# GinZhu/RDST

Hardware: AMD Instinct MI355X
Metric: SR patches/sec fwd+bwd, RDST-E1 x4 64->256 (higher is better)
Workload: dtype bf16; 1 GPU; RDST-E1 x4 (RDST_E1_OASIS_example_SRx4.ini), 1x64x64 LR patches -> 256x256, step = fwd + L1 + bwd + flat-bucket grad all-reduce + Adam; global_batch=32, per_gpu_batch=32, parallelism=dp1, hip_graph=True, grad_bucket_bytes=17859844

## Files before the change

rdst_amd/csrc/lin3_mfma.hip:

```cpp
#include "linear.h"
#include "lds_dma.h"
#include "mfma.h"
#include "pack.h"

namespace {

constexpr int L3_TT = 128;

__global__ void __launch_bounds__(256) lin3_pack_kernel(const float* __restrict__ W, const float* __restrict__ gamma,
                                                        const float* __restrict__ beta, const float* __restrict__ bias,
                                                        bf16* __restrict__ wp, float* __restrict__ sb, int N, int K, int ksteps,
                                                        int ntiles, float s) {
  lin3_pack_block((int)blockIdx.x, W, gamma, beta, bias, wp, sb, N, K, ksteps, ntiles, s);
}

struct L3Args {
  const bf16* X; int64_t ldx; int x_bytes;
  const bf16* Wp; const float* sb;
  const bf16* R; int64_t ldr; int r_bytes;
  bf16* Y; int64_t ldy;
  float* stats;
  int M, N, ntiles;
};

constexpr int l3_nw(int NT) { return (NT >= 4 && NT <= 12) ? NT : 8; }

template <int K, int NT, bool LN, bool RES>
struct L3Cfg {
  static constexpr int KSTEPS = (K + 15) / 16;
  static constexpr int XS = lds_kstep_stride(K), XSLOTS = XS / 16, XD = (2 * K + 15) / 16;
  static constexpr int TP = (L3_TT * XSLOTS + 63) / 64, TILEB = TP * 1024;
  static constexpr int RS = RES ? NT * 64 + 16 : 0, RSLOTS = RS / 16, RP = RES ? (L3_TT * RSLOTS + 63) / 64 : 0, RTILEB = RP * 1024;
  static constexpr int WGCU = l3_nw(NT) > 8 ? 1 : 2;
  static constexpr int NBUF = RES ? 1 : (WGCU == 1 ? 4 : 2);
  static constexpr int NW = l3_nw(NT);
  static constexpr int NTHR = 64 * NW;
  static constexpr int ITEMS = NT * 4, NJ = (ITEMS + NW - 1) / NW;
  static constexpr int PERIOD = NT / ce_gcd(NW, NT), ND = NJ < PERIOD ? NJ : PERIOD;
  static constexpr int CNT = (TP + NW - 1) / NW + (RES ? (RP + NW - 1) / NW : 0);
  static constexpr int R_OFF = NBUF * TILEB;
  static constexpr int STAT_OFF = R_OFF + NBUF * RTILEB;
  static constexpr int SB_OFF = STAT_OFF + NBUF * L3_TT * 2 * 4;
  static constexpr int SMEM = SB_OFF + (2 * NT * 32 * 4 + 1023) / 1024 * 1024;
  static_assert(SMEM <= 160 * 1024, "LDS");
  static_assert(CNT * (NBUF - 1) < 64, "vmcnt is a 6-bit counter");
  static_assert(TP >= NW && (!RES || RP >= NW), "every wave owns at least one piece of a tile");
};

template <int K, int NT, bool LN, bool RES>
__global__ void __launch_bounds__(64 * l3_nw(NT), l3_nw(NT) > 8 ? 1 : (2 * l3_nw(NT) + 3) / 4) lin3_kernel(const L3Args p) {
  using CF = L3Cfg<K, NT, LN, RES>;
  constexpr int KSTEPS = CF::KSTEPS, XS = CF::XS, NBUF = CF::NBUF, ND = CF::ND, NJ = CF::NJ, NW = CF::NW, NTHR = CF::NTHR;
  extern __shared__ __attribute__((aligned(16))) char smem[];
  const int tid = threadIdx.x, lane = tid & 63, r = lane & 31, h = lane >> 5;
  const int wave = __builtin_amdgcn_readfirstlane(tid >> 6);
  float* statL = reinterpret_cast<float*>(smem + CF::STAT_OFF);
  const float* sbL = reinterpret_cast<const float*>(smem + CF::SB_OFF);

  const u32x4s_t rsx = dma_rsrc(p.X, (uint32_t)p.x_bytes), rsr = dma_rsrc(RES ? (const void*)p.R : (const void*)p.X, (uint32_t)p.r_bytes),
                 rsb = dma_rsrc(p.sb, 2 * NT * 32 * 4);
  const uint32_t lds0 = lds_base(smem);
  const int grid = gridDim.x;
  u32x4v_t wfr[ND][KSTEPS];
#pragma unroll
  for (int jd = 0; jd < ND; ++jd) {
    const int nt = (wave + NW * jd) % NT;
#pragma unroll
    for (int ks = 0; ks < KSTEPS; ++ks) {
      const char* src = reinterpret_cast<const char*>(p.Wp) + (((int64_t)nt * KSTEPS + ks) * 64 + lane) * 16;
      frag_load(wfr[jd][ks], src);
    }
  }
  {
    constexpr int NSBP = (2 * NT * 32 * 4 + 1023) / 1024;
    const int pc = wave % NSBP;
    lds_dma16(rsb, __builtin_amdgcn_readfirstlane(lds0 + (uint32_t)(CF::SB_OFF + pc * 1024)), pc * 1024 + lane * 16);
  }
  constexpr int CNT = CF::CNT;
  auto issue_round = [&](int tile0) {
#pragma unroll
    for (int b = 0; b < NBUF; ++b) {
      const int tile = tile0 + b * grid;
#pragma unroll
      for (int i = 0; i < (CF::TP + NW - 1) / NW; ++i) {
        int q = wave + NW * i;
        q = q < CF::TP ? q : q - NW;
        const int sidx = q * 64 + lane;
        const int tok = sidx / CF::XSLOTS, sl = sidx - tok * CF::XSLOTS;
        const int grow = tile * L3_TT + tok;
        const bool ok = tile < p.ntiles && tok < L3_TT && sl < CF::XD && grow < p.M;
        lds_dma16(rsx, __builtin_amdgcn_readfirstlane(lds0 + (uint32_t)(b * CF::TILEB + q * 1024)),
            ok ? grow * ((int)p.ldx * 2) + sl * 16 : p.x_bytes);
      }
      if constexpr (RES) {
#pragma unroll
        for (int i = 0; i < (CF::RP + NW - 1) / NW; ++i) {
          int q = wave + NW * i;
          q = q < CF::RP ? q : q - NW;
          const int sidx = q * 64 + lane;
          const int tok = sidx / CF::RSLOTS, sl = sidx - tok * CF::RSLOTS;
          const int grow = tile * L3_TT + tok;
          const bool ok = tile < p.ntiles && tok < L3_TT && sl * 8 < p.N && grow < p.M;
          lds_dma16(rsr, __builtin_amdgcn_readfirstlane(lds0 + (uint32_t)(CF::R_OFF + b * CF::RTILEB + q * 1024)),
              ok ? grow * ((int)p.ldr * 2) + sl * 16 : p.r_bytes);
        }
      }
    }
  };

  for (int tile0 = blockIdx.x; tile0 < p.ntiles; tile0 += grid * NBUF) {
    issue_round(tile0);
#pragma unroll 1
    for (int b = 0; b < NBUF; ++b) {
      const int tile = tile0 + b * grid;
      if (tile >= p.ntiles) break;
      switch (NBUF - 1 - b) {
        case 3: wait_vmcnt<CNT * 3>(); break;
        case 2: wait_vmcnt<CNT * 2>(); break;
        case 1: wait_vmcnt<CNT * 1>(); break;
        default: wait_vmcnt<0>(); break;
      }
#pragma unroll
      for (int jd = 0; jd < ND; ++jd)
#pragma unroll
        for (int ks = 0; ks < KSTEPS; ++ks) frag_pin(wfr[jd][ks]);
      __syncthreads();
      const char* tb = smem + b * CF::TILEB;
      const char* rb = smem + CF::R_OFF + b * CF::RTILEB;
      float* st = statL + b * L3_TT * 2;
      if constexpr (LN) {
        for (int tok = tid >> 2; tok < L3_TT; tok += NTHR / 4) {
          const int part = tid & 3;
          constexpr int NSL = (CF::XD + 3) / 4;
          float xv[NSL][8];
          float sum = 0.f;
#pragma unroll
          for (int i = 0; i < NSL; ++i) {
            const int sl = part + 4 * i;
            const Pack16 q = *reinterpret_cast<const Pack16*>(tb + tok * XS + (sl < CF::XD ? sl : 0) * 16);
            Mma<bf16>::unpack(q, xv[i]);
#pragma unroll
            for (int e = 0; e < 8; ++e) {
              const bool valid = sl < CF::XD && sl * 8 + e < K;
              xv[i][e] = valid ? xv[i][e] : 0.f;
              sum += xv[i][e];
            }
          }
          sum += __shfl_xor(sum, 1, 64);
          sum += __shfl_xor(sum, 2, 64);
          const float mean = sum * (1.0f / K);
          float sq = 0.f;
#pragma unroll
          for (int i = 0; i < NSL; ++i) {
            const int sl = part + 4 * i;
#pragma unroll
            for (int e = 0; e < 8; ++e) {
              const bool valid = sl < CF::XD && sl * 8 + e < K;
              const float d = xv[i][e] - mean;
              sq = valid ? fmaf(d, d, sq) : sq;
            }
          }
          sq += __shfl_xor(sq, 1, 64);
          sq += __shfl_xor(sq, 2, 64);
          const float rstd = rsqrtf(sq * (1.0f / K) + 1e-5f);
          if (part == 0) {
            st[tok * 2] = mean;
            st[tok * 2 + 1] = rstd;
            const int grow = tile * L3_TT + tok;
            if (grow < p.M) *reinterpret_cast<float2*>(p.stats + (int64_t)grow * 2) = make_float2(mean, rstd);
          }
        }
        __syncthreads();
      }
#pragma unroll
      for (int jd = 0; jd < ND; ++jd)
#pragma unroll 1
      for (int j = jd; j < NJ; j += ND) {
        const int item = wave + NW * j;
        if (item >= CF::ITEMS) break;
        const int nt = item % NT, tt = item / NT;
        const int tok = tt * 32 + r;
        const int grow = tile * L3_TT + tok;
        f32x16 acc;
#pragma unroll
        for (int v = 0; v < 16; ++v) acc[v] = 0.f;
        const char* brow = tb + tok * XS + h * 16;
#pragma unroll
        for (int ks = 0; ks < KSTEPS; ++ks) {
          Pack16 bq = *reinterpret_cast<const Pack16*>(brow + ks * 32);
          if (K % 16 != 0 && ks == KSTEPS - 1) {
            constexpr int c0 = K % 16 < 8 ? K % 16 : 8, c1 = K % 16 > 8 ? K % 16 - 8 : 0;
#pragma unroll
            for (int d = 0; d < 4; ++d) bq.w[d] = (2 * d < (h ? c1 : c0)) ? bq.w[d] : 0u;
          }
          acc = __builtin_amdgcn_mfma_f32_32x32x16_bf16(__builtin_bit_cast(bf16x8_t, wfr[jd][ks]), __builtin_bit_cast(bf16x8_t, bq), acc, 0, 0, 0);
        }
        float mean = 0.f, rstd = 1.f;
        if constexpr (LN) {
          const float2 mr = *reinterpret_cast<const float2*>(st + tok * 2);
          mean = mr.x; rstd = mr.y;
        }
        const float nrm = -rstd * mean;
#pragma unroll
        for (int g4 = 0; g4 < 4; ++g4) {
          const int n0 = nt * 32 + 8 * g4 + 4 * h;
          const float4 S4 = *reinterpret_cast<const float4*>(sbL + n0);
          const float4 B4 = *reinterpret_cast<const float4*>(sbL + NT * 32 + n0);
          if constexpr (LN) {
            acc[4 * g4] = fmaf(rstd, acc[4 * g4], fmaf(nrm, S4.x, B4.x));
            acc[4 * g4 + 1] = fmaf(rstd, acc[4 * g4 + 1], fmaf(nrm, S4.y, B4.y));
            acc[4 * g4 + 2] = fmaf(rstd, acc[4 * g4 + 2], fmaf(nrm, S4.z, B4.z));
            acc[4 * g4 + 3] = fmaf(rstd, acc[4 * g4 + 3], fmaf(nrm, S4.w, B4.w));
          } else {
            acc[4 * g4] += B4.x; acc[4 * g4 + 1] += B4.y; acc[4 * g4 + 2] += B4.z; acc[4 * g4 + 3] += B4.w;
          }
          if constexpr (RES) {
            const u32x2_a4 rr = *reinterpret_cast<const u32x2_a4*>(rb + tok * CF::RS + n0 * 2);
            acc[4 * g4] += bf16lo(rr.x); acc[4 * g4 + 1] += bf16hi(rr.x);
            acc[4 * g4 + 2] += bf16lo(rr.y); acc[4 * g4 + 3] += bf16hi(rr.y);
          }
        }
        if (grow < p.M) {
#pragma unroll
          for (int gp = 0; gp < 2; ++gp) {
            float c8[8];
#pragma unroll
            for (int e = 0; e < 4; ++e) {
              const auto sw = __builtin_amdgcn_permlane32_swap(__float_as_uint(acc[8 * gp + e]), __float_as_uint(acc[8 * gp + 4 + e]),
                                                               false, false);
              c8[e] = __uint_as_float(sw[0]);
              c8[4 + e] = __uint_as_float(sw[1]);
            }
            const int cb = nt * 32 + 8 * (2 * gp + h);
            const int nv = p.N - cb;
            if (nv <= 0) continue;
            bf16* yp = p.Y + (grow * (int)p.ldy + cb);
            if (nv >= 8) {
              u32x4_a4 u;
              u.x = pack_bf16x2(c8[0], c8[1]); u.y = pack_bf16x2(c8[2], c8[3]);
              u.z = pack_bf16x2(c8[4], c8[5]); u.w = pack_bf16x2(c8[6], c8[7]);
              *reinterpret_cast<u32x4_a4*>(yp) = u;
            } else {
#pragma unroll
              for (int d = 0; d < 3; ++d)
                if (2 * d + 2 <= nv) *reinterpret_cast<uint32_t*>(yp + 2 * d) = pack_bf16x2(c8[2 * d], c8[2 * d + 1]);
            }
          }
        }
      }
    }
    __syncthreads();
  }
}

template <int K, int NT, bool LN, bool RES>
int launch_l3(L3Args& p, hipStream_t st, const char* what) {
  using CF = L3Cfg<K, NT, LN, RES>;
  p.ntiles = (p.M + L3_TT - 1) / L3_TT;
  int grid = (p.ntiles + CF::NBUF - 1) / CF::NBUF;
  if (grid > 256 * CF::WGCU) grid = 256 * CF::WGCU;
  auto kern = lin3_kernel<K, NT, LN, RES>;
  return rdst_launch(kern, dim3((unsigned)grid), dim3(CF::NTHR), CF::SMEM, st, what, p);
}

}

int lin3_pack_launch(const float* W, const float* gamma, const float* beta, const float* bias, void* out, int N, int K, float s,
                     hipStream_t st) {
  const int nt = (N + 31) / 32, ks = (K + 15) / 16;
  bf16* wp = reinterpret_cast<bf16*>(out);
  float* sb = reinterpret_cast<float*>(reinterpret_cast<char*>(out) + (size_t)nt * ks * 1024);
  const int nfr = nt * ks * 64, nb1 = (nfr + 255) / 256, nb2 = (nt * 32 + 3) / 4;
  hipLaunchKernelGGL(lin3_pack_kernel, dim3((unsigned)(nb1 + nb2)), dim3(256), 0, st, W, gamma, beta, bias, wp, sb, N, K, ks, nt, s);
  return rdst_launch_status("lin3_pack");
}

size_t lin3_pack_bytes(int K, int N) {
  const int nt = (N + 31) / 32, ks = (K + 15) / 16;
  return (size_t)nt * ks * 1024 + (size_t)2 * nt * 32 * 4 + 256;
}

int lin3_kind(int K, int N, bool ln, bool res, int in_act) {
  if (in_act || !(K == 60 || K == 90 || K == 120)) return 0;
  if (ln && !res && N == 3 * K) return 1;
  if (!ln && res && N == K) return 2;
  if (ln && !res && N == 30) return 3;
  return 0;
}

int lin3_fwd_bf16(const bf16* X, int64_t ldx, const float* ln_w, const float* ln_b, int in_act, const float* Wt, const float* bias,
                  const bf16* R, int64_t ldr, bf16* Y, int64_t ldy, float* stats, int64_t M, int K, int N, float s, void* wpack,
                  bool prepacked, hipStream_t st) {
  if (!wpack || ((uintptr_t)wpack & 15) || !Wt || M <= 0) return RDST_ENOTSUP;
  const int kind = lin3_kind(K, N, ln_w != nullptr, R != nullptr, in_act);
  if (!kind) return RDST_ENOTSUP;
  if (((uintptr_t)X & 3) || (ldx & 1) || ((uintptr_t)Y & 3) || (ldy & 1) || (R && (((uintptr_t)R & 3) || (ldr & 1)))) return RDST_ENOTSUP;
  const int64_t xb = ((M - 1) * ldx + K) * 2;
  if (xb >= (1ll << 31) || M * ldy * 2 >= (1ll << 31) || (R && M * ldr * 2 >= (1ll << 31))) return RDST_ENOTSUP;
  const int nt = (N + 31) / 32, ks = (K + 15) / 16;
  bf16* wp = reinterpret_cast<bf16*>(wpack);
  float* sb = reinterpret_cast<float*>(reinterpret_cast<char*>(wpack) + (size_t)nt * ks * 1024);
  if (!prepacked)
    if (int rc = lin3_pack_launch(Wt, ln_w, ln_b, bias, wpack, N, K, s, st)) return rc;
  L3Args p{};
  p.X = X; p.ldx = ldx; p.x_bytes = (int)xb; p.Wp = wp; p.sb = sb; p.R = R; p.ldr = ldr;
  p.r_bytes = R ? (int)(((M - 1) * ldr + N) * 2) : 0; p.Y = Y; p.ldy = ldy; p.stats = stats;
  p.M = (int)M; p.N = N;
#define L3_CASE(KK)                                                                                   \
  if (K == KK) {                                                                                      \
    if (kind == 1) return launch_l3<KK, (3 * KK + 31) / 32, true, false>(p, st, "lin3_qkv");           \
    if (kind == 2) return launch_l3<KK, (KK + 31) / 32, false, true>(p, st, "lin3_proj");              \
    return launch_l3<KK, 1, true, false>(p, st, "lin3_tail");                                          \
  }
  L3_CASE(60) L3_CASE(90) L3_CASE(120)
#undef L3_CASE
  return RDST_ENOTSUP;
}
```

rdst_amd/csrc/linear.h:

```cpp
#pragma once
#include "common.h"

template <typename T>
int linear_fwd_mfma(const T* X, int64_t ldx, const float* ln_w, const float* ln_b, int in_act, const float* Wt,
                    const float* bias, const T* R, int64_t ldr, T* Y, int64_t ldy, float* stats, int64_t M, int K,
                    int N, float s, bool split, hipStream_t st);
template <typename T>
int linear_dgrad_mfma(const T* X, int64_t ldx, bool has_ln, int in_act, const float* Wt, const T* dY, int64_t lddy,
                      T* dX, int64_t lddx, const T* acc, int64_t ldacc, float* dA, int64_t M, int K, int N, float s,
                      bool split, hipStream_t st);
template <typename T>
int linear_wgrad_mfma(const T* X, int64_t ldx, const float* ln_w, const float* ln_b, const float* stats, int in_act,
                      const T* dY, int64_t lddy, float* dW, float* dbias, const WsSlab& slab, int64_t M, int K, int N, float s,
                      bool split, hipStream_t st);

constexpr int kLinWgradSplits = 96;
inline int linear_wgrad_max_wgs(int N) { return N <= 128 ? 4 * kCUs : N <= 192 ? 2 * kCUs : kCUs; }
struct LinBwdWs {
  float* dA;
  float* G;
  WsSlab slabW;
  WsSlab small;
  size_t bytes;
};
inline LinBwdWs lin_bwd_layout(void* base, int64_t M, int K, int N, bool ln, bool linear) {
  WsCarver c(base);
  LinBwdWs w{};
  const size_t g = (size_t)N * (K + 1), da = ln ? (size_t)M * K : 0;
  w.dA = c.take<float>(da);
  w.G = ln && linear && g <= da ? w.dA : nullptr;
  const int64_t rows = linear ? linear_wgrad_max_wgs(N) : 0;
  const size_t gen = linear ? (size_t)kLinWgradSplits * N * K : 0, per_wg = (size_t)rows * g;
  w.slabW = WsSlab{c.take<float>(gen > per_wg ? gen : per_wg), rows, (int64_t)g};
  w.small = ws_take_slab(c, kSmallBlocks, N > 2 * K ? N : 2 * K);
  c.take<float>(2 * (size_t)K + kWsSlackFloats);
  w.bytes = c.bytes();
  return w;
}

template <typename T>
int linear_dgrad_ln_mfma(const T* X, int64_t ldx, const float* stats, const float* gamma, const float* Wt, const T* dY,
                         int64_t lddy, T* dX, int64_t lddx, const T* acc, int64_t ldacc, const WsSlab& slab, int* nslab,
                         int64_t M, int K, int N, float s, hipStream_t st);
template <typename T>
int linear_wgrad_ln_mfma(const T* X, int64_t ldx, const float* ln_w, const float* ln_b, const float* stats, const float* Wt,
                         const T* dY, int64_t lddy, float* dW, float* dbias, float* dln_w, float* dln_b, const WsSlab& slab,
                         float* G, int64_t M, int K, int N, float s, bool split, hipStream_t st);
template <typename T>
int linear_dgrad_ln2_mfma(const T* X, int64_t ldx, const float* stats, const float* gamma, const float* Wt, const T* dY,
                          int64_t lddy, T* dX, int64_t lddx, const T* acc, int64_t ldacc, int64_t M, int K, int N, float s,
                          bool split, hipStream_t st);
int wgrad_ln_finish_launch(const float* G, const float* Wt, const float* ln_w, const float* ln_b, int N, int K, float s,
                           float* dW, float* dbias, float* dln_w, float* dln_b, hipStream_t st);
int wgrad_sum_launch(const float* slab, int nwg, int tot, float* G, hipStream_t st);
int wgrad_reduce_launch(const float* slab, int nwg, int N, int K, float s, float* dW, float* dbias, hipStream_t st);
int linear_ln_bwd_fused_bf16(const bf16* X, int64_t ldx, const float* ln_w, const float* ln_b, const float* stats,
                             const float* Wt, const bf16* dY, int64_t lddy, bf16* dX, int64_t lddx, const bf16* acc,
                             int64_t ldacc, float* dW, float* dbias, float* dln_w, float* dln_b, const WsSlab& slab, float* G,
                             int64_t M, int K, int N, float s, hipStream_t st, const bf16* acc2 = nullptr, int64_t ldacc2 = 0);
int lnlin3_bwd_bf16(const bf16* X, int64_t ldx, const float* ln_w, const float* stats, const float* Wt, const bf16* dY,
                    int64_t lddy, bf16* dX, int64_t lddx, const bf16* acc, int64_t ldacc, const bf16* acc2, int64_t ldacc2,
                    const WsSlab& slab, int64_t slab_stride, int64_t M, int K, int N, int* grid_out, hipStream_t st);

size_t lin3_pack_bytes(int K, int N);
int lin3_kind(int K, int N, bool ln, bool res, int in_act);
int lin3_fwd_bf16(const bf16* X, int64_t ldx, const float* ln_w, const float* ln_b, int in_act, const float* Wt, const float* bias,
                  const bf16* R, int64_t ldr, bf16* Y, int64_t ldy, float* stats, int64_t M, int K, int N, float s, void* wpack,
                  bool prepacked, hipStream_t st);
int lin3_pack_launch(const float* W, const float* gamma, const float* beta, const float* bias, void* out, int N, int K, float s,
                     hipStream_t st);
size_t mlp3_pack_bytes(int C, int hid);
bool mlp3_fwd_shape(int C, int hid);
int mlp3_fwd_bf16(const bf16* X, int64_t ldx, const float* ln_w, const float* ln_b, const float* W1, const float* b1, const float* W2,
                  const float* b2, bf16* Y, int64_t ldy, float* stats, int64_t M, int C, int hid, void* wpack, bool prepacked,
                  hipStream_t st);

int lin3x_kind(int K, int N, bool ln, bool res, int in_act);
int lin3x_fwd_f32(const float* X, int64_t ldx, const float* ln_w, const float* ln_b, int in_act, const float* Wt, const float* bias,
                  const float* R, int64_t ldr, float* Y, int64_t ldy, float* stats, int64_t M, int K, int N, float s, void* wpack,
                  bool prepacked, hipStream_t st);
int lin3x_pack_launch(const float* W, const float* gamma, const float* beta, const float* bias, void* out, int N, int K, float s,
                      hipStream_t st);
int lnlin3x_bwd_kind(int K, int N, bool ln, int in_act);
int lnlin3x_bwd_f32(const float* X, int64_t ldx, const float* ln_w, const float* ln_b, const float* stats, int in_act, const float* Wt,
                    const float* dY, int64_t lddy, float* dX, int64_t lddx, const float* acc, int64_t ldacc, const float* acc2,
                    int64_t ldacc2, float* dW, float* dbias, float* dln_w, float* dln_b, const WsSlab& slab, float* G, int64_t M, int K, int N,
                    float s, hipStream_t st);
```

Measured before the change: 1929 patches/s.

## Add persistent register-pipelined LN+linear kernel for the 30-wide tail projection

Adds a dedicated persistent-wave forward kernel for the LayerNorm+linear tail case (N=30). It keeps the packed weights in registers, prefetches the next 32-row X tile into registers while the current tile is staged in LDS, computes LN statistics and a single MFMA chain, and writes the bf16 outputs through permlane swaps. The kernel replaces the generic lin3 tail path when available. It adds a new code path with env-controlled occupancy (2 blocks per CU by default) and more edge-handling complexity.

```diff
diff --git a/rdst_amd/csrc/lin3_mfma.hip b/rdst_amd/csrc/lin3_mfma.hip
--- a/rdst_amd/csrc/lin3_mfma.hip
+++ b/rdst_amd/csrc/lin3_mfma.hip
@@ -302,6 +302,10 @@
   float* sb = reinterpret_cast<float*>(reinterpret_cast<char*>(wpack) + (size_t)nt * ks * 1024);
   if (!prepacked)
     if (int rc = lin3_pack_launch(Wt, ln_w, ln_b, bias, wpack, N, K, s, st)) return rc;
+  if (kind == 3) {
+    const int rc = tail30_fwd_bf16(X, ldx, wp, sb, Y, ldy, stats, M, K, st);
+    if (rc != RDST_ENOTSUP) return rc;
+  }
   L3Args p{};
   p.X = X; p.ldx = ldx; p.x_bytes = (int)xb; p.Wp = wp; p.sb = sb; p.R = R; p.ldr = ldr;
   p.r_bytes = R ? (int)(((M - 1) * ldr + N) * 2) : 0; p.Y = Y; p.ldy = ldy; p.stats = stats;
diff --git a/rdst_amd/csrc/linear.h b/rdst_amd/csrc/linear.h
--- a/rdst_amd/csrc/linear.h
+++ b/rdst_amd/csrc/linear.h
@@ -69,6 +69,8 @@
                   bool prepacked, hipStream_t st);
 int lin3_pack_launch(const float* W, const float* gamma, const float* beta, const float* bias, void* out, int N, int K, float s,
                      hipStream_t st);
+int tail30_fwd_bf16(const bf16* X, int64_t ldx, const bf16* wp, const float* sb, bf16* Y, int64_t ldy, float* stats, int64_t M, int K,
+                    hipStream_t st);
 size_t mlp3_pack_bytes(int C, int hid);
 bool mlp3_fwd_shape(int C, int hid);
 int mlp3_fwd_bf16(const bf16* X, int64_t ldx, const float* ln_w, const float* ln_b, const float* W1, const float* b1, const float* W2,
diff --git a/rdst_amd/csrc/tail30_mfma.hip b/rdst_amd/csrc/tail30_mfma.hip
--- /dev/null
+++ b/rdst_amd/csrc/tail30_mfma.hip
@@ -0,0 +1,215 @@
+#include "linear.h"
+#include "lds_dma.h"
+#include "mfma.h"
+#include <stdlib.h>
+
+namespace {
+
+constexpr int T30_NW = 4;
+
+struct T30FArgs {
+  const bf16* X; int ldxb;
+  const bf16* Wp; const float* sb;
+  bf16* Y; int ldy;
+  float* stats;
+  int M, nsub;
+};
+
+template <int K>
+struct T30F {
+  static constexpr int KSTEPS = (K + 15) / 16;
+  static constexpr int REM = K % 16;
+  static constexpr int V1 = REM == 0 ? 8 : REM > 8 ? REM - 8 : 0;
+  static_assert(REM == 0 || REM >= 8, "lane half 0 of the last k-step is whole");
+  static_assert(V1 % 2 == 0, "whole dwords");
+};
+
+template <int E>
+struct T30Flat {
+  static constexpr int RB = 2 * E, XD = (RB + 15) / 16;
+  static constexpr bool SHIFT = RB % 16 != 0;
+  static constexpr int LASTO = RB - 16;
+  static constexpr int RPI = 64 / XD, NI = (32 + RPI - 1) / RPI;
+};
+template <int E>
+__device__ __forceinline__ void t30_flat_load(const void* base, size_t ldb, int row0, int M, int lane, u32x4_a4 (&v)[T30Flat<E>::NI]) {
+  using F = T30Flat<E>;
+  const int lr0 = lane / F::XD, sl = lane - lr0 * F::XD;
+  const int lr = lr0 < F::RPI ? lr0 : 0;
+  const int so = (F::SHIFT && sl == F::XD - 1) ? F::LASTO : sl * 16;
+#pragma unroll
+  for (int j = 0; j < F::NI; ++j) {
+    int row = row0 + j * F::RPI + lr;
+    row = row < M ? row : M - 1;
+    v[j] = *reinterpret_cast<const u32x4_a4*>(reinterpret_cast<const char*>(base) + (size_t)row * ldb + so);
+  }
+}
+template <int E>
+__device__ __forceinline__ void t30_flat_stage(char* area, int LD, int lane, const u32x4_a4 (&v)[T30Flat<E>::NI]) {
+  using F = T30Flat<E>;
+  const int lr = lane / F::XD, sl = lane - lr * F::XD;
+  const bool last = F::SHIFT && sl == F::XD - 1;
+  const int so = last ? F::LASTO : sl * 16;
+#pragma unroll
+  for (int j = 0; j < F::NI; ++j) {
+    const int rl = j * F::RPI + lr;
+    if (lr < F::RPI && rl < 32) {
+      char* dst = area + rl * LD + so;
+      if (last) {
+        uint32_t* d = reinterpret_cast<uint32_t*>(dst);
+        d[0] = v[j].x; d[1] = v[j].y; d[2] = v[j].z; d[3] = v[j].w;
+      } else {
+        *reinterpret_cast<u32x4_a4*>(dst) = v[j];
+      }
+    }
+  }
+}
+template <int K>
+__device__ __forceinline__ void t30_lds_row(const char* row, int h, u32x4_a4 (&x)[T30F<K>::KSTEPS]) {
+  using CF = T30F<K>;
+#pragma unroll
+  for (int ks = 0; ks < CF::KSTEPS; ++ks) {
+    x[ks] = *reinterpret_cast<const u32x4_a4*>(row + ks * 32 + h * 16);
+    if (ks == CF::KSTEPS - 1 && CF::V1 < 8) {
+      const uint32_t a[4] = {x[ks].x, x[ks].y, x[ks].z, x[ks].w};
+      uint32_t m[4];
+#pragma unroll
+      for (int d = 0; d < 4; ++d) m[d] = (h && 2 * d >= CF::V1) ? 0u : a[d];
+      x[ks].x = m[0]; x[ks].y = m[1]; x[ks].z = m[2]; x[ks].w = m[3];
+    }
+  }
+}
+
+template <int K>
+__global__ void __launch_bounds__(64 * T30_NW) tail30_fwd_kernel(const T30FArgs p) {
+  using CF = T30F<K>;
+  constexpr int KSTEPS = CF::KSTEPS;
+  __shared__ __attribute__((aligned(16))) float sbL[64];
+  const int tid = threadIdx.x, lane = tid & 63, r = lane & 31, h = lane >> 5;
+  const int wave = __builtin_amdgcn_readfirstlane(tid >> 6);
+  if (tid < 64) sbL[tid] = p.sb[tid];
+  u32x4_a4 wfr[KSTEPS];
+#pragma unroll
+  for (int ks = 0; ks < KSTEPS; ++ks)
+    wfr[ks] = *reinterpret_cast<const u32x4_a4*>(reinterpret_cast<const char*>(p.Wp) + (ks * 64 + lane) * 16);
+  __syncthreads();
+
+  constexpr int XS = lds_kstep_stride(K);
+  __shared__ __attribute__((aligned(16))) char stage[T30_NW * 32 * XS];
+  char* area = stage + wave * (32 * XS);
+  const int nwaves = gridDim.x * T30_NW;
+  int sub = blockIdx.x * T30_NW + wave;
+  u32x4_a4 xf[T30Flat<K>::NI];
+  t30_flat_load<K>(p.X, (size_t)p.ldxb, sub * 32, p.M, lane, xf);
+  for (; sub < p.nsub; sub += nwaves) {
+    __builtin_amdgcn_wave_barrier();
+    t30_flat_stage<K>(area, XS, lane, xf);
+    __builtin_amdgcn_wave_barrier();
+    asm volatile("" ::: "memory");
+    t30_flat_load<K>(p.X, (size_t)p.ldxb, (sub + nwaves) * 32, p.M, lane, xf);
+    u32x4_a4 x[1][KSTEPS];
+    t30_lds_row<K>(area + r * XS, h, x[0]);
+    {
+      constexpr int u = 0;
+      const int grow = sub * 32 + r;
+      float sa = 0.f, sb2 = 0.f;
+#pragma unroll
+      for (int ks = 0; ks < KSTEPS; ++ks) {
+        float f[8];
+        unpack8(x[u][ks], f);
+#pragma unroll
+        for (int e = 0; e < 8; ++e) {
+          if (ks & 1) sb2 += f[e];
+          else sa += f[e];
+        }
+      }
+      sa += __shfl_xor(sa, 32, 64);
+      sb2 += __shfl_xor(sb2, 32, 64);
+      const float mean = (sa + sb2) * (1.0f / K);
+      float qa = 0.f, qb = 0.f;
+#pragma unroll
+      for (int ks = 0; ks < KSTEPS; ++ks) {
+        float f[8];
+        unpack8(x[u][ks], f);
+#pragma unroll
+        for (int e = 0; e < 8; ++e) {
+          const bool valid = ks * 16 + h * 8 + e < K;
+          const float d = f[e] - mean;
+          if (ks & 1) qb = valid ? fmaf(d, d, qb) : qb;
+          else qa = valid ? fmaf(d, d, qa) : qa;
+        }
+      }
+      qa += __shfl_xor(qa, 32, 64);
+      qb += __shfl_xor(qb, 32, 64);
+      const float rstd = rsqrtf((qa + qb) * (1.0f / K) + 1e-5f);
+      if (h == 0 && grow < p.M) *reinterpret_cast<float2*>(p.stats + (int64_t)grow * 2) = make_float2(mean, rstd);
+
+      f32x16 acc;
+#pragma unroll
+      for (int v = 0; v < 16; ++v) acc[v] = 0.f;
+#pragma unroll
+      for (int ks = 0; ks < KSTEPS; ++ks)
+        acc = __builtin_amdgcn_mfma_f32_32x32x16_bf16(__builtin_bit_cast(bf16x8_t, wfr[ks]), __builtin_bit_cast(bf16x8_t, x[u][ks]), acc, 0, 0, 0);
+      const float nrm = -rstd * mean;
+#pragma unroll
+      for (int g4 = 0; g4 < 4; ++g4) {
+        const int n0 = 8 * g4 + 4 * h;
+        const float4 S4 = *reinterpret_cast<const float4*>(sbL + n0);
+        const float4 B4 = *reinterpret_cast<const float4*>(sbL + 32 + n0);
+        acc[4 * g4] = fmaf(rstd, acc[4 * g4], fmaf(nrm, S4.x, B4.x));
+        acc[4 * g4 + 1] = fmaf(rstd, acc[4 * g4 + 1], fmaf(nrm, S4.y, B4.y));
+        acc[4 * g4 + 2] = fmaf(rstd, acc[4 * g4 + 2], fmaf(nrm, S4.z, B4.z));
+        acc[4 * g4 + 3] = fmaf(rstd, acc[4 * g4 + 3], fmaf(nrm, S4.w, B4.w));
+      }
+      if (grow < p.M) {
+#pragma unroll
+        for (int gp = 0; gp < 2; ++gp) {
+          float c8[8];
+#pragma unroll
+          for (int e = 0; e < 4; ++e) {
+            const auto sw = __builtin_amdgcn_permlane32_swap(__float_as_uint(acc[8 * gp + e]), __float_as_uint(acc[8 * gp + 4 + e]),
+                                                             false, false);
+            c8[e] = __uint_as_float(sw[0]);
+            c8[4 + e] = __uint_as_float(sw[1]);
+          }
+          const int cb = 8 * (2 * gp + h);
+          bf16* yp = p.Y + ((size_t)grow * (size_t)p.ldy + cb);
+          if (cb + 8 <= 30) {
+            u32x4_a4 u4;
+            u4.x = pack_bf16x2(c8[0], c8[1]); u4.y = pack_bf16x2(c8[2], c8[3]);
+            u4.z = pack_bf16x2(c8[4], c8[5]); u4.w = pack_bf16x2(c8[6], c8[7]);
+            *reinterpret_cast<u32x4_a4*>(yp) = u4;
+          } else {
+#pragma unroll
+            for (int d = 0; d < 3; ++d) *reinterpret_cast<uint32_t*>(yp + 2 * d) = pack_bf16x2(c8[2 * d], c8[2 * d + 1]);
+          }
+        }
+      }
+    }
+  }
+}
+
+template <int K>
+int t30_fwd_launch(T30FArgs& p, int per_cu, hipStream_t st) {
+  const int groups = (p.nsub + T30_NW - 1) / T30_NW;
+  const int cap = kCUs * per_cu;
+  auto kern = tail30_fwd_kernel<K>;
+  return rdst_launch(kern, dim3((unsigned)(groups < cap ? groups : cap)), dim3(64 * T30_NW), 0, st, "tail30_fwd", p);
+}
+
+}
+
+int tail30_fwd_bf16(const bf16* X, int64_t ldx, const bf16* wp, const float* sb, bf16* Y, int64_t ldy, float* stats, int64_t M, int K,
+                    hipStream_t st) {
+  static int off = -1, percu = -1;
+  if (off < 0) { const char* e = rdst_dbg_getenv("RDST_T30_OFF"); off = e ? atoi(e) : 0; }
+  if (percu < 0) { const char* e = rdst_dbg_getenv("RDST_T30_FWD_PERCU"); percu = e && atoi(e) > 0 ? atoi(e) : 2; }
+  if ((off & 1) || !stats || M <= 0) return RDST_ENOTSUP;
+  T30FArgs p{};
+  p.X = X; p.ldxb = (int)(ldx * 2); p.Wp = wp; p.sb = sb; p.Y = Y; p.ldy = (int)ldy; p.stats = stats;
+  p.M = (int)M; p.nsub = (int)((M + 31) / 32);
+  if (K == 60) return t30_fwd_launch<60>(p, percu, st);
+  if (K == 90) return t30_fwd_launch<90>(p, percu, st);
+  if (K == 120) return t30_fwd_launch<120>(p, percu, st);
+  return RDST_ENOTSUP;
+}
```

Result: no change. 1927 patches/s (-0.1%).
